# nicooff/omp_amg

Hardware: AMD Instinct MI355X
Metric: AMG setup rows/sec + RAP SpGEMM nnz/sec at 1/2/4/8 MI355X (higher is better)
Workload: dtype f64

## Files before the change

omp_amg_amd/__init__.py:

```python
from __future__ import annotations

import ctypes as C
import os
import subprocess

import numpy as np

from . import abi

HERE = os.path.dirname(os.path.abspath(__file__))
LIB_PATH = os.path.join(HERE, "libomp_amg_amd.so")
_lib = None


class AmgdStats(C.Structure):
    _fields_ = [("t_total_ms", C.c_double), ("t_build_ms", C.c_double),
                ("t_coarsen_ms", C.c_double), ("t_smoother_ms", C.c_double),
                ("t_interp_ms", C.c_double), ("t_rap_ms", C.c_double),
                ("t_copy_ms", C.c_double), ("rap_kernel_ms", C.c_double),
                ("rap_out_nnz", C.c_uint64), ("rap_bytes", C.c_uint64),
                ("rows0", C.c_uint64), ("nnz0", C.c_uint64),
                ("nlevels", C.c_uint32), ("ub_events", C.c_uint32),
                ("peak_bytes", C.c_size_t), ("spmv_kernel_ms", C.c_double),
                ("spmv_bytes", C.c_uint64), ("spmv_bytes_strict", C.c_uint64),
# ... 64 lines not shown
        L.amgd_test_kry_mdot_n.argtypes = [C.c_void_p, C.c_void_p, C.c_uint64, C.c_uint64, C.c_int, C.c_void_p,
                                           C.c_void_p]
        L.amgd_test_kry_update_n.argtypes = [C.c_void_p, C.c_void_p, C.c_void_p, C.c_uint64, C.c_uint64, C.c_int,
                                             C.c_void_p, C.c_void_p]
        L.amgd_test_kry_mdot.argtypes = [C.c_void_p, C.c_void_p, C.c_uint64, C.c_uint64, C.c_int, C.c_void_p]
        L.amgd_test_kry_update.argtypes = [C.c_void_p, C.c_void_p, C.c_void_p, C.c_uint64, C.c_uint64, C.c_int,
                                           C.c_void_p]
        L.amgd_test_vc_level_n.argtypes = [C.POINTER(HCsr), C.POINTER(HCsr), C.POINTER(HCsr), C.c_void_p,
                                           C.c_uint32, C.c_double, C.c_void_p, C.c_void_p, C.c_void_p,
                                           C.c_int, C.c_int]
        L.amgd_test_vc_restrict_n.argtypes = [C.POINTER(HCsr), C.c_void_p, C.c_void_p, C.c_int, C.c_int]
        L.amgd_test_vc_mrhs_k.argtypes = [C.c_int]
        L.amgd_test_vc_mrhs_family.argtypes = [C.c_int]
        L.amgd_test_vc_row_max.argtypes = [C.c_uint32]
        L.amgd_test_vc_level.argtypes = [C.POINTER(HCsr), C.POINTER(HCsr), C.POINTER(HCsr), C.c_void_p,
                                         C.c_uint32, C.c_double, C.c_void_p, C.c_void_p, C.c_int,
                                         C.c_void_p, C.c_void_p, C.c_void_p]
        L.amgd_test_vc_restrict.argtypes = [C.POINTER(HCsr), C.c_void_p, C.c_void_p, C.c_int]
        L.amgd_hier_rows.argtypes = [C.c_void_p, C.POINTER(C.c_uint32), C.POINTER(C.c_uint32)]
        L.amgd_hier_rows.restype = C.c_int
        L.amgd_solve_comm_stats.argtypes = [C.POINTER(C.c_uint64), C.POINTER(C.c_uint64)]
        L.amgd_test_vc_halo.argtypes = [C.c_int]
        L.amgd_test_vc_repl.argtypes = [C.c_int64]
        L.amgd_test_vc_restrict_map.argtypes = [C.POINTER(HCsr), C.c_void_p, C.c_void_p, C.c_uint32,
                                                C.c_void_p, C.c_int]
        L.amgd_test_vc_halo_xch.argtypes = [C.POINTER(HCsr), C.c_void_p, C.c_void_p, C.c_void_p]
        L.amgd_test_vc_fused.argtypes = [C.c_int]
        L.amgd_test_vc_tail.argtypes = [C.c_int]
        L.amgd_test_vc_coop.argtypes = [C.c_int]
        L.amgd_dev_alloc.argtypes = [C.c_size_t]
        L.amgd_dev_alloc.restype = C.c_void_p
        L.amgd_dev_free.argtypes = [C.c_void_p]
        L.amgd_dev_upload.argtypes = [C.c_void_p, C.c_void_p, C.c_size_t]
        L.amgd_dev_download.argtypes = [C.c_void_p, C.c_void_p, C.c_size_t]
        L.amgd_test_csr.argtypes = [C.c_int, C.POINTER(HCsr), C.POINTER(HCsr), C.c_double,
                                    C.c_double, C.POINTER(HCsr)]
        L.amgd_test_spmv.argtypes = [C.POINTER(HCsr), C.c_void_p, C.c_double, C.c_void_p,
                                     C.c_double, C.c_void_p]
        L.amgd_test_spmv_f.argtypes = [C.POINTER(HCsr), C.c_void_p, C.c_double, C.c_void_p,
                                       C.c_double, C.c_void_p, C.c_void_p]
        L.amgd_test_spmv_rows.argtypes = [C.POINTER(HCsr), C.c_void_p, C.c_uint32, C.c_void_p,
                                          C.c_void_p]
        L.amgd_test_spmv_sl_min.argtypes = [C.c_int64]
        L.amgd_test_build.argtypes = [C.c_uint64, C.c_void_p, C.c_void_p, C.c_void_p,
                                      C.POINTER(HCsr)]
        L.amgd_test_math.argtypes = [C.c_int, C.c_uint64, C.c_void_p, C.c_void_p, C.c_void_p]
        L.amgd_test_free.argtypes = [C.POINTER(HCsr)]
        L.amgd_test_dot.argtypes = [C.c_int, C.c_uint64, C.c_void_p, C.c_void_p, C.c_int, C.c_int]
        L.amgd_test_dot.restype = C.c_double
        L.amgd_test_lmop_mode.argtypes = [C.c_int]
        L.amgd_test_spgemm_flat.argtypes = [C.c_int]
        L.amgd_test_spgemm_win.argtypes = [C.c_int]
        L.amgd_test_qf_reuse.argtypes = [C.c_int]
        L.amgd_test_sg_pattern.argtypes = [C.c_int]
        L.amgd_test_lmop_wave.argtypes = [C.c_int]
        L.amgd_test_lmop_small.argtypes = [C.c_int]
        L.amgd_test_lmop_stats.argtypes = [C.POINTER(C.c_uint64), C.c_int]
        L.amgd_test_lmop_prune.argtypes = [C.c_int]
        L.amgd_test_qf_sparse.argtypes = [C.c_int]
        L.amgd_test_qf_stats.argtypes = [C.POINTER(C.c_uint64)]
        L.amgd_test_qf_coop_lds.argtypes = [C.c_int]
        L.amgd_test_qf_split.argtypes = [C.c_int]
        L.amgd_test_mv_long.argtypes = [C.c_int64]
        L.amgd_test_fs_long.argtypes = [C.c_int64]
        L.amgd_test_spmv_rw.argtypes = [C.c_int]
        L.amgd_test_spmv_pair.argtypes = [C.c_int]
        L.amgd_test_spmv_rw_bounds.argtypes = [C.c_int, C.c_int]
        L.amgd_test_d2h_poll.argtypes = [C.c_int]
        L.amgd_test_fs_amx.argtypes = [C.c_int]
        L.amgd_test_qa_tile.argtypes = [C.c_int]
        L.amgd_test_qa_huge.argtypes = [C.c_int]
        L.amgd_test_qa_small.argtypes = [C.c_int]
        L.amgd_test_spmv_shard_calls.restype = C.c_uint64
        L.amgd_test_route_stats.argtypes = [C.POINTER(C.c_uint64), C.c_int]
        L.amgd_comm_rccl_uid.argtypes = [C.c_char_p]
        L.amgd_comm_rccl_uid.restype = C.c_int
        L.amgd_comm_init_rccl.argtypes = [C.c_int, C.c_int, C.c_char_p]
        L.amgd_comm_init_rccl.restype = C.c_int
        L.amgd_comm_init_host.argtypes = [C.c_int, C.c_int, C.c_void_p, C.c_void_p]
        L.amgd_comm_init_host.restype = C.c_int
        L.amgd_comm_init_sim.argtypes = [C.c_int]
        L.amgd_comm_init_sim.restype = C.c_int
        L.amgd_comm_set_min_work.argtypes = [C.c_double]
        L.amgd_comm_stats.argtypes = [C.POINTER(C.c_uint64), C.POINTER(C.c_uint64),
                                      C.POINTER(C.c_double)]
        _lib = L
    return _lib


def init(device: int = 0) -> None:
    L = lib()
    if L.amgd_init(device) != 0:
        raise RuntimeError("omp_amg_amd: no usable HIP device: " + L.amgd_error().decode())


def amg_setup(Ai, Aj, Av, *, seed: int = 1) -> abi.Hierarchy:
    init()
    return abi.run_setup(lib(), Ai, Aj, Av, seed=seed, quiet=False)


def stats() -> dict:
    st = AmgdStats()
    lib().amgd_get_stats(C.byref(st))
    out = {}
    for f, _ in AmgdStats._fields_:
        v = getattr(st, f)
# ... 446 lines not shown

def lmop_stats(reset: bool = True) -> dict:
    out = (C.c_uint64 * 5)()
    lib().amgd_test_lmop_stats(out, int(reset))
    return {"fast": out[0], "general": out[1], "dirty_prefix": out[2], "misses": out[3],
            "pruned": out[4]}


def lmop_prune(n: int) -> None:
    lib().amgd_test_lmop_prune(int(n))


def spgemm_dr_sort(on: int) -> None:
    lib().amgd_test_spgemm_dr_sort(int(on))


def spat_inc(on: int) -> None:
    lib().amgd_test_spat_inc(int(on))


def skel_tr(on: int) -> None:
    lib().amgd_test_skel_tr(int(on))


def fuse_arr(on: int) -> None:
    lib().amgd_test_fuse_arr(int(on))


def spat_stats() -> dict:
    out = (C.c_uint64 * 3)()
    lib().amgd_test_spat_stats(out)
    return {"incremental": out[0], "whole": out[1], "same": out[2]}


def spgemm_sym(mode: int) -> None:
    lib().amgd_test_spgemm_sym(int(mode))


def spgemm_sym_stats() -> dict:
    L = lib()
    k, r = C.c_uint64(), C.c_uint64()
    L.amgd_test_spgemm_sym_stats(C.byref(k), C.byref(r))
    return {"kept": k.value, "reused": r.value}


def spgemm_win(w: int) -> None:
    lib().amgd_test_spgemm_win(int(w))


def qf_reuse(on: int) -> None:
    lib().amgd_test_qf_reuse(int(on))


def lmop_wave(n: int) -> None:
    lib().amgd_test_lmop_wave(int(n))


def sg_pattern(on: int) -> None:
    lib().amgd_test_sg_pattern(int(on))


def qa_small(on: int) -> None:
    lib().amgd_test_qa_small(int(on))


def lmop_qq_budget(nbytes: int) -> None:
    L = lib()
    L.amgd_test_lmop_qq_budget.argtypes = [C.c_int64]
    L.amgd_test_lmop_qq_budget(int(nbytes))


def _hcsr_any(M):
    h = _to_hcsr(M.row_off, M.col if len(M.col) else np.zeros(1), M.a if len(M.a) else np.zeros(1),
                 M.rn, M.cn)
    h.nnz = int(M.row_off[-1])
    return h


def test_qapply(Wt: abi.Csr, A: abi.Csr, Bt: abi.Csr, u, lam):
    init()
    L = lib()
    L.amgd_test_qapply.argtypes = [C.POINTER(HCsr), C.POINTER(HCsr), C.POINTER(HCsr), C.c_void_p,
                                   C.c_void_p, C.c_void_p]
    hs = [_hcsr_any(M) for M in (Wt, A, Bt)]
    u = np.ascontiguousarray(u, dtype=np.float64)
    lam = np.ascontiguousarray(lam, dtype=np.float64)
    assert len(u) == Wt.rn and len(lam) == Wt.cn
    out = np.zeros(int(Wt.row_off[-1]) + 1)
    rc = L.amgd_test_qapply(C.byref(hs[0]), C.byref(hs[1]), C.byref(hs[2]), u.ctypes.data,
                            lam.ctypes.data, out.ctypes.data)
    if rc != 0:
        raise RuntimeError(f"amgd_test_qapply failed rc={rc}")
    return out[:-1]


def test_lmop(S: abi.Csr, Wskel: abi.Csr, A: abi.Csr, u):
    init()
    L = lib()
    L.amgd_test_lmop.argtypes = [C.POINTER(HCsr), C.POINTER(HCsr), C.POINTER(HCsr), C.c_void_p,
                                 C.c_void_p]
    hs = [_hcsr_any(M) for M in (S, Wskel, A)]
    u = np.ascontiguousarray(u, dtype=np.float64)
    assert len(u) == Wskel.cn
    out = np.zeros(int(S.row_off[-1]) + 1)
    rc = L.amgd_test_lmop(C.byref(hs[0]), C.byref(hs[1]), C.byref(hs[2]), u.ctypes.data, out.ctypes.data)
    if rc != 0:
# ... 580 lines not shown
```

omp_amg_amd/csrc/amgd_interp.hip:

```cpp
#include <hip/hip_runtime.h>
#include <cstring>
#include <rocprim/device/device_radix_sort.hpp>

#include <cfloat>
#include <cstdio>
#include <cstdlib>
#include <algorithm>
#include <vector>

#include "amgd.h"
#include "amgd_dev.h"

__device__ __forceinline__ uint64_t tri(uint64_t i) { return i * (i + 1) / 2; }

__device__ __forceinline__ double row_lookup(const uint32_t *col, const double *a, uint64_t a0,
                                             uint64_t a1, uint32_t j) {
  uint64_t lo = a0, hi = a1;
  while (lo < hi) {
    uint64_t mid = (lo + hi) >> 1;
    if (col[mid] < j) lo = mid + 1;
    else hi = mid;
  }
  return (lo < a1 && col[lo] == j) ? a[lo] : 0.0;
}
// ... 161 lines not shown
#pragma unroll
    for (int q = 0; q < QB; q++) {
      uint32_t j = j0 + q;
      if (j < k && j >= i) y += r[q] * s2[j];
    }
  }
  return y;
}

__global__ __launch_bounds__(256) void k_qfactor_mid(const uint32_t *rows, uint32_t nrows,
                                                     const uint64_t *wro, const uint32_t *wcol,
                                                     const uint64_t *aro, const uint32_t *acol,
                                                     const double *aa, const uint64_t *qoff,
                                                     double *Q) {
  __shared__ double s1[1024], s2[1024], qk[1024];
  __shared__ uint32_t Qs[1024];
  __shared__ double sh_al;
  const int t = threadIdx.x, lane = t & 63;
  for (uint32_t r = blockIdx.x; r < nrows; r += gridDim.x) {
    const uint32_t c = rows[r];
    const uint64_t w0 = wro[c];
    const uint32_t nz = (uint32_t)(wro[c + 1] - w0);
    for (uint32_t m = t; m < nz; m += 256) Qs[m] = wcol[w0 + m];
    double *U = Q + qoff[c];
    __syncthreads();
    for (uint32_t k = 0; k < nz; k++) {
      const uint32_t sk = Qs[k];
      gather_s1<256>(s1, Qs, k, acol, aa, aro[sk], aro[sk + 1]);
      __syncthreads();
      for (uint32_t i = t; i < k; i += 256) s2[i] = seq_dot_batched(U + tri(i), s1, i + 1);
      __syncthreads();
      for (uint32_t ib = t - lane; ib < k; ib += 256) {
        const uint32_t i = ib + lane;
        double y = mv_ut_lane(U, s2, ib, i, k);
        if (i < k) qk[i] = y;
      }
      __syncthreads();
      if (t == 0) {
        double al = s1[k];
        for (uint32_t m = 0; m < k; m++) al -= s1[m] * qk[m];
        sh_al = -1.0 / sqrt(al);
      }
      __syncthreads();
      const double al = sh_al;
      double *out = U + tri(k);
      for (uint32_t i = t; i < k; i += 256) out[i] = qk[i] * al;
      if (t == 0) out[k] = -al;
      __syncthreads();
    }
  }
}

#define QB2 16
template <int NZMAX, int B, int NTT = 256>
__global__ __launch_bounds__(NTT) void k_qfactor_blk(const uint32_t *rows, uint32_t nrows,
                                                     const uint64_t *wro, const uint32_t *wcol,
                                                     const uint64_t *aro, const uint32_t *acol,
                                                     const double *aa, const uint64_t *qoff,
                                                     double *Q) {
  constexpr uint32_t NT = NTT, RPT = (NZMAX + NT - 1) / NT, PAD = NZMAX + 16;
  __shared__ uint32_t Qs[NZMAX];
  __shared__ double S1[B * PAD], S2[B * PAD], qk[PAD];
  __shared__ double sh_al;
  const uint32_t t = threadIdx.x, lane = t & 63;
  for (uint32_t r = blockIdx.x; r < nrows; r += gridDim.x) {
    const uint32_t c = rows[r];
    const uint64_t w0 = wro[c];
    const uint32_t nz = (uint32_t)(wro[c + 1] - w0);
    for (uint32_t m = t; m < nz; m += NT) Qs[m] = wcol[w0 + m];
    double *U = Q + qoff[c];
    __syncthreads();
    for (uint32_t k0 = 0; k0 < nz; k0 += B) {
      const uint32_t bn = min((uint32_t)B, nz - k0);
      for (uint32_t b = 0; b < bn; b++)
        for (uint32_t m = t; m <= k0 + b; m += NT) S1[b * PAD + m] = 0.0;
      uint64_t ra0[B];
      uint32_t rlen[B], spre[B + 1], lpre[B + 1];
      uint32_t look_cost = 0, scan_cost = 0;
      spre[0] = lpre[0] = 0;
#pragma unroll
      for (int b = 0; b < B; b++) {
        ra0[b] = 0;
        rlen[b] = 0;
        if ((uint32_t)b < bn) {
          const uint32_t k = k0 + b, sk = Qs[k];
          ra0[b] = aro[sk];
          rlen[b] = (uint32_t)(aro[sk + 1] - ra0[b]);
          const uint32_t lg_len = 32 - __clz(rlen[b] | 1), lg_k = 32 - __clz(k + 1);
          look_cost += (k + 1) * lg_len * 4;
          scan_cost += rlen[b] * (4 + lg_k);
        }
        spre[b + 1] = spre[b] + rlen[b];
        lpre[b + 1] = lpre[b] + ((uint32_t)b < bn ? k0 + b + 1 : 0u);
      }
      __syncthreads();
      if (look_cost < scan_cost) {
        for (uint32_t fl = t; fl < lpre[B]; fl += NT) {
          uint32_t b = 0;
#pragma unroll
          for (int q = 1; q < B; q++) b += fl >= lpre[q] ? 1u : 0u;
          const uint32_t m = fl - lpre[b];
          S1[b * PAD + m] = row_lookup(acol, aa, ra0[b], ra0[b] + rlen[b], Qs[m]);
        }
      } else {
        for (uint32_t fl = t; fl < spre[B]; fl += NT) {
          uint32_t b = 0;
#pragma unroll
          for (int q = 1; q < B; q++) b += fl >= spre[q] ? 1u : 0u;
          const uint64_t a0 = ra0[b], e = a0 + (fl - spre[b]);
          const uint32_t k = k0 + b;
          const uint32_t j = acol[e];
          if (e > a0 && acol[e - 1] == j) continue;
          uint32_t lo = 0, hi = k + 1;
          while (lo < hi) {
            const uint32_t mid = (lo + hi) >> 1;
            if (Qs[mid] < j) lo = mid + 1;
            else hi = mid;
          }
          if (lo <= k && Qs[lo] == j) S1[b * PAD + lo] = aa[e];
        }
      }
      __syncthreads();
      for (uint32_t i = t; i < k0; i += NT) {
        double acc[B];
#pragma unroll
        for (int b = 0; b < B; b++) acc[b] = 0.0;
        const double *Ui = U + tri(i);
        for (uint32_t j0 = 0; j0 <= i; j0 += QB2) {
          double u[QB2];
#pragma unroll
          for (int q = 0; q < QB2; q++) u[q] = (j0 + q <= i) ? Ui[j0 + q] : 0.0;
#pragma unroll
          for (int q = 0; q < QB2; q++)
            if (j0 + q <= i) {
#pragma unroll
              for (int b = 0; b < B; b++) acc[b] += u[q] * S1[b * PAD + j0 + q];
            }
        }
#pragma unroll
        for (int b = 0; b < B; b++)
          if ((uint32_t)b < bn) S2[b * PAD + i] = acc[b];
      }
      __syncthreads();
      double part[RPT][B];
#pragma unroll
      for (uint32_t rr = 0; rr < RPT; rr++) {
        const uint32_t ib = (t - lane) + rr * NT, i = ib + lane;
#pragma unroll
        for (int b = 0; b < B; b++) part[rr][b] = 0.0;
        for (uint32_t j0 = ib; j0 < k0; j0 += QB2) {
          double u[QB2];
#pragma unroll
          for (int q = 0; q < QB2; q++) {
            const uint32_t j = j0 + q;
            u[q] = (j < k0 && j >= i) ? U[tri(j) + i] : 0.0;
          }
#pragma unroll
          for (int q = 0; q < QB2; q++) {
            const uint32_t j = j0 + q;
            if (j < k0 && j >= i) {
#pragma unroll
              for (int b = 0; b < B; b++) part[rr][b] += u[q] * S2[b * PAD + j];
            }
          }
        }
      }
#pragma unroll
      for (int b = 0; b < B; b++) {
        if ((uint32_t)b < bn) {
          const uint32_t k = k0 + b;
#pragma unroll
          for (uint32_t rr = 0; rr < RPT; rr++) {
            const uint32_t i = t + rr * NT;
            if (i < k) {
              double y = i < k0 ? part[rr][b] : 0.0;
              for (uint32_t j = max(i, k0); j < k; j++) y += U[tri(j) + i] * S2[b * PAD + j];
              qk[i] = y;
            }
          }
          __syncthreads();
          if (t == 0) {
            const double *s1 = S1 + b * PAD;
            double al = s1[k];
            for (uint32_t m0 = 0; m0 < k; m0 += LB) {
              double x[LB], y[LB];
#pragma unroll
              for (int q = 0; q < LB; q++) { x[q] = s1[m0 + q]; y[q] = qk[m0 + q]; }
#pragma unroll
              for (int q = 0; q < LB; q++)
                if (m0 + q < k) al -= x[q] * y[q];
            }
            sh_al = -1.0 / sqrt(al);
          }
          __syncthreads();
          const double al = sh_al;
          double *out = U + tri(k);
          for (uint32_t i = t; i < k; i += NT) out[i] = qk[i] * al;
          if (t == 0) out[k] = -al;
          if (t < bn - 1 - b) {
            const double *s1 = S1 + (b + 1 + t) * PAD;
            double v = 0;
            for (uint32_t j0 = 0; j0 < k; j0 += LB) {
              double x[LB], y[LB];
#pragma unroll
              for (int q = 0; q < LB; q++) { x[q] = qk[j0 + q]; y[q] = s1[j0 + q]; }
#pragma unroll
              for (int q = 0; q < LB; q++)
                if (j0 + q < k) v += (x[q] * al) * y[q];
            }
            v += (-al) * s1[k];
            S2[(b + 1 + t) * PAD + k] = v;
          }
          __syncthreads();
        }
      }
    }
  }
}

__device__ __forceinline__ void grid_sync(unsigned *bar, unsigned nblocks, unsigned &gen) {
  __threadfence();
  __syncthreads();
  if (threadIdx.x == 0) {
    unsigned a = atomicAdd(&bar[0], 1u);
    if (a == nblocks - 1) {
      atomicExch(&bar[0], 0u);
      __threadfence();
      atomicAdd(&bar[1], 1u);
    } else {
      while (__hip_atomic_load(&bar[1], __ATOMIC_ACQUIRE, __HIP_MEMORY_SCOPE_AGENT) == gen)
        __builtin_amdgcn_s_sleep(1);
    }
  }
  __syncthreads();
  __threadfence();
  gen++;
}

#define QF_COOP_MAX 8192
template <bool LDS>
__global__ __launch_bounds__(64) void k_qfactor_coop(uint32_t c, const uint64_t *wro,
                                                     const uint32_t *wcol, const uint64_t *aro,
                                                     const uint32_t *acol, const double *aa,
                                                     const uint64_t *qoff, double *Q,
                                                     double *s1b, double *s2, double *qk,
                                                     unsigned *bar) {
  extern __shared__ double xs[];
  __shared__ double sh_al;
  const uint32_t lane = threadIdx.x, G = gridDim.x;
  const uint32_t gt = blockIdx.x * 64 + lane, GT = G * 64;
  const uint64_t w0 = wro[c];
  const uint32_t nz = (uint32_t)(wro[c + 1] - w0);
  const uint32_t *Qj = wcol + w0;
  double *U = Q + qoff[c];
  double *xa = xs, *xb = xs + nz;
  unsigned gen = 0;
  for (uint32_t k = 0; k <= nz; k++) {
    if (k > 0) {
      const uint32_t kp = k - 1;
      const double *s1p = s1b + (uint64_t)(kp & 1) * nz;
      if (LDS) {
// ... 233 lines not shown
}
__global__ void k_max_nz(const uint64_t *wro, uint32_t rn, unsigned long long *mx) {
  unsigned long long m = 0;
  GRID_STRIDE(c, rn) m = max(m, (unsigned long long)(wro[c + 1] - wro[c]));
  atomicMax(mx, m);
}

struct RowSplit {
  uint32_t *sl, *bl;
  unsigned ns, nb;
  uint64_t maxnz;
};
static RowSplit split_rows(const dcsr *Wt, uint32_t cap, uint32_t cb, uint32_t ce) {
  RowSplit rs;
  const uint64_t L = (uint64_t)Wt->rn + 1;
  rs.sl = (uint32_t *)amgd_alloc(2 * L * 4);
  rs.bl = rs.sl + L;
  unsigned *cnt = (unsigned *)amgd_alloc(32);
  amgd_memset(cnt, 0, 32);
  if (ce > cb) {
    k_bin_nz<<<grid_for(ce - cb), 256, 0, amgd_s()>>>(Wt->ro, cb, ce, BinLim{{cap}}, 2, rs.sl, cnt, L);
    k_max_nz<<<grid_for(Wt->rn), 256, 0, amgd_s()>>>(Wt->ro, Wt->rn, (unsigned long long *)(cnt + 4));
  }
  unsigned h[8];
  amgd_d2h(h, cnt, 32);
  amgd_free(cnt);
  rs.ns = h[0];
  rs.nb = h[1];
  uint64_t mx;
  memcpy(&mx, &h[4], 8);
  rs.maxnz = mx;
  return rs;
}
static void free_split(RowSplit &rs) { amgd_free(rs.sl); }

static int g_qf_sparse = -1;
static bool g_qf_sparse_forced = false;
static int qf_sparse_mode() {
  if (g_qf_sparse < 0) {
    const char *e = getenv("AMGD_QF_SPARSE");
    g_qf_sparse = e ? atoi(e) : 1;
    g_qf_sparse_forced = e != nullptr;
  }
  return g_qf_sparse;
}
static int qf_blocked() {
  static int b = -1;
  if (b < 0) {
    const char *e = getenv("AMGD_QF_BLOCKED");
    b = e ? atoi(e) : 1;
  }
  return b;
}
static uint32_t g_coop_lds_max = QF_COOP_MAX;
extern "C" void amgd_qfactor_set_coop_lds(int m) { g_coop_lds_max = m < 0 ? QF_COOP_MAX : (uint32_t)m; }
static unsigned long g_qf_stats[3];
extern "C" void amgd_qfactor_set_sparse(int m) {
  g_qf_sparse = m;
  g_qf_sparse_forced = m >= 0 && m != 1;
}
extern "C" void amgd_qfactor_stats(unsigned long *st) {
  st[0] = g_qf_stats[0];
  st[1] = g_qf_stats[1];
  st[2] = g_qf_stats[2];
  g_qf_stats[0] = g_qf_stats[1] = g_qf_stats[2] = 0;
}
#define QF_T0 32
#define QF_T1 64
#define QF_T2 128
#define QF_T3 1024
__global__ void k_cc_init(const uint32_t *Qj, uint32_t nz, uint32_t *pos, uint32_t *lab) {
  GRID_STRIDE(k, nz) {
    pos[Qj[k]] = (uint32_t)k;
    lab[k] = (uint32_t)k;
  }
}
__global__ void k_cc_reset(const uint32_t *Qj, uint32_t nz, uint32_t *pos) {
  GRID_STRIDE(k, nz) pos[Qj[k]] = 0xffffffffu;
}
__global__ void k_cc_hook(const uint32_t *Qj, uint32_t nz, const uint64_t *aro,
                          const uint32_t *acol, const uint32_t *pos, uint32_t *lab,
                          unsigned *changed) {
  GRID_STRIDE(k, nz) {
    const uint32_t r = Qj[k];
    uint32_t m = lab[k];
    for (uint64_t e = aro[r]; e < aro[r + 1]; e++) {
      const uint32_t p = pos[acol[e]];
      if (p != 0xffffffffu) m = min(m, lab[p]);
    }
    bool ch = false;
    for (uint64_t e = aro[r]; e < aro[r + 1]; e++) {
      const uint32_t p = pos[acol[e]];
      if (p == 0xffffffffu) continue;
      const uint32_t lp = lab[p];
      if (m < lp) { atomicMin(&lab[lp], m); atomicMin(&lab[p], m); ch = true; }
    }
    const uint32_t lk = lab[k];
    if (m < lk) { atomicMin(&lab[lk], m); atomicMin(&lab[k], m); ch = true; }
    if (ch) *changed = 1u;
  }
}
__global__ void k_cc_init_iota(uint32_t nz, uint32_t *lab) { GRID_STRIDE(k, nz) lab[k] = (uint32_t)k; }
__global__ void k_cc_jump(uint32_t nz, uint32_t *lab) {
  GRID_STRIDE(k, nz) {
    uint32_t l = lab[k];
    while (lab[l] != l) l = lab[l];
// ... 248 lines not shown
      return g_qf_split_depth > 0 && nz <= 8192 && !g_qf_sparse_forced ? 0 : sp0;
    };
    std::vector<uint32_t> bigs;
    for (uint32_t c : big) {
      const uint32_t nz = (uint32_t)(ro[c + 1] - ro[c]);
      if (!qfactor_split(c, Wt, A, ro[c], nz, Q + qo[c])) bigs.push_back(c);
    }
    big.swap(bigs);
    if (!big.empty()) amgd_sync();
    for (uint32_t c : big) {
      uint32_t nz = (uint32_t)(ro[c + 1] - ro[c]);
      bignz.push_back(nz);
      const int sp = sp_of(nz);
      if (!sp) {
        bigstat.push_back(nullptr);
        launch_coop(c, nz);
        continue;
      }
      const uint64_t tn = (uint64_t)nz * (nz + 1) / 2;
      const uint32_t cap = sp == 2 ? nz + 8 : (uint32_t)std::min<uint64_t>(tn, 1u << 24);
      const size_t nd = (size_t)nz * 3 + cap, nu = (size_t)nz * 6 + (size_t)cap * 3 + 2;
      char *mem = (char *)amgd_alloc(nd * 8 + nu * 4 + 64);
      coop_bufs.push_back(mem);
      QsBuf qb;
      qb.s1 = (double *)mem;
      qb.s2 = qb.s1 + nz;
      qb.qk = qb.s2 + nz;
      qb.uval = qb.qk + nz;
      uint32_t *u = (uint32_t *)(qb.uval + cap);
      qb.m2 = u;
      qb.m3 = u + nz;
      qb.L2 = u + 2 * (size_t)nz;
      qb.chead = u + 3 * (size_t)nz;
      qb.ctail = u + 4 * (size_t)nz;
      qb.rowptr = u + 5 * (size_t)nz;
      qb.ucol = u + 6 * (size_t)nz + 1;
      qb.urow = qb.ucol + cap;
      qb.nxt = qb.urow + cap;
      qb.status = qb.nxt + cap;
      qb.cap = cap;
      HIPCK(hipMemsetAsync(mem, 0, (size_t)nz * 3 * 8, s2));
      HIPCK(hipMemsetAsync(qb.m2, 0, (size_t)nz * 3 * 4, s2));
      HIPCK(hipMemsetAsync(qb.chead, 0xff, (size_t)nz * 2 * 4, s2));
      k_fill_negzero<<<grid_for(tn), 256, 0, s2>>>(Q + qo[c], tn);
      k_qfactor_sparse<256><<<1, 256, 0, s2>>>(c, Wt->ro, Wt->col, A->ro, A->col, A->a, qoff, Q, qb);
      KCHECK();
      bigstat.push_back(qb.status);
    }
    HIPCK(hipEventRecord(ev2, s2));
  }
  if (hn[0])
    k_qfactor_lds<QF_T0, 64><<<(int)std::min<unsigned>(hn[0], 65536u), 64, 0, s>>>(
        lists, hn[0], Wt->ro, Wt->col, A->ro, A->col, A->a, qoff, Q);
  if (hn[1])
    k_qfactor_blk<QF_T1, 4, 64><<<(int)std::min<unsigned>(hn[1], 65536u), 64, 0, s>>>(
        lists + L, hn[1], Wt->ro, Wt->col, A->ro, A->col, A->a, qoff, Q);
  if (hn[2])
    k_qfactor_blk<QF_T2, 4, 128><<<(int)std::min<unsigned>(hn[2], 65536u), 128, 0, s>>>(
        lists + 2 * L, hn[2], Wt->ro, Wt->col, A->ro, A->col, A->a, qoff, Q);
  if (qf_blocked()) {
    if (hn[3])
      k_qfactor_blk<256, 4><<<(int)std::min<unsigned>(hn[3], 8192u), 256, 0, s>>>(
          lists + 3 * L, hn[3], Wt->ro, Wt->col, A->ro, A->col, A->a, qoff, Q);
    if (hn[4]) amgd_route_hit(AMGD_R_QF_T512);
    if (hn[5]) amgd_route_hit(AMGD_R_QF_T1024);
    if (hn[4])
      k_qfactor_blk<512, 4><<<(int)std::min<unsigned>(hn[4], 8192u), 256, 0, s>>>(
          lists + 4 * L, hn[4], Wt->ro, Wt->col, A->ro, A->col, A->a, qoff, Q);
    if (hn[5])
      k_qfactor_blk<QF_T3, 4><<<(int)std::min<unsigned>(hn[5], 8192u), 256, 0, s>>>(
          lists + 5 * L, hn[5], Wt->ro, Wt->col, A->ro, A->col, A->a, qoff, Q);
  } else {
    for (int q = 3; q < 6; q++)
      if (hn[q])
        k_qfactor_mid<<<(int)std::min<unsigned>(hn[q], 8192u), 256, 0, s>>>(
            lists + q * L, hn[q], Wt->ro, Wt->col, A->ro, A->col, A->a, qoff, Q);
  }
  KCHECK();
  if (hn[HUGE]) {
    bool redo = false;
    for (size_t q = 0; q < big.size(); q++) {
      if (!bigstat[q]) continue;
      unsigned st = 0;
      HIPCK(hipMemcpyAsync(&st, bigstat[q], 4, hipMemcpyDeviceToHost, s2));
      HIPCK(hipStreamSynchronize(s2));
      if (st) {
        amgd_sync();
        launch_coop(big[q], bignz[q]);
        redo = true;
      }
      g_qf_stats[st ? 1 : 0]++;
    }
    if (redo) HIPCK(hipEventRecord(ev2, s2));
    HIPCK(hipStreamWaitEvent(s, ev2, 0));
    for (void *p : coop_bufs) amgd_free(p);
  }
  if (sglog) {
    amgd_sync();
    fprintf(stderr, "qfactor cols %u nnz %lu tiers %u/%u/%u/%u/%u/%u/%u (huge nz %u) Q %lu  %.2f ms\n",
            rn, (unsigned long)Wt->nnz, hn[0], hn[1], hn[2], hn[3], hn[4], hn[5], hn[6],
            bignz.empty() ? 0u : bignz[0], (unsigned long)tot, (amgd_wtime() - t_start) * 1e3);
  }
  amgd_free(lists); amgd_free(cnt);
}

__global__ void k_qcost(const uint64_t *wro, uint32_t rn, uint64_t *cost, const uint8_t *skip) {
  GRID_STRIDE(c, rn) {
    uint64_t nz = wro[c + 1] - wro[c];
    cost[c] = (skip && skip[c] ? nz * nz / 8 : nz <= 1024 ? nz * nz * nz : nz * nz * 1024) + 1;
  }
}
#define QF_SHARD_MIN (1ull << 30)
static int g_qf_reuse = -1;
static int qf_reuse_on() {
  if (g_qf_reuse < 0) { const char *e = getenv("AMGD_QF_REUSE"); g_qf_reuse = e && *e ? atoi(e) : 1; }
  return g_qf_reuse;
}
extern "C" void amgd_qfactor_set_reuse(int on) { g_qf_reuse = on < 0 ? -1 : on; }
extern "C" void amgd_qfactor_reuse_stats(uint64_t *reused, uint64_t *factored) {
  *reused = g_qf_reused; *factored = g_qf_factored;
}
extern "C" double *amgd_qfactor(const dcsr *Wt, const dcsr *A, uint64_t **qoff_out,
                                uint64_t *qtotal) {
  return amgd_qfactor_reuse(Wt, A, qoff_out, qtotal, nullptr, nullptr, nullptr);
}
extern "C" double *amgd_qfactor_reuse(const dcsr *Wt, const dcsr *A, uint64_t **qoff_out,
                                      uint64_t *qtotal, const dcsr *Wp, const double *Qp,
                                      const uint64_t *qpoff) {
  hipStream_t s = amgd_s();
  const uint32_t rn = Wt->rn;
// ... 1575 lines not shown
```

omp_amg_amd/csrc/amgd_testapi.c:

```c
#include <stdlib.h>
#include <string.h>

#include "amgd.h"

#define API __attribute__((visibility("default")))

typedef struct { uint32_t rn, cn; uint64_t nnz; uint64_t *ro; uint32_t *col; double *a; } hcsr;

static dcsr *up(const hcsr *H) {
  dcsr *A = dcsr_new(H->rn, H->cn, H->nnz);
  amgd_h2d(A->ro, H->ro, ((size_t)H->rn + 1) * 8);
  amgd_h2d(A->col, H->col, H->nnz * 4);
  amgd_h2d(A->a, H->a, H->nnz * 8);
  return A;
}
static void down(const dcsr *A, hcsr *H) {
  H->rn = A->rn; H->cn = A->cn; H->nnz = A->nnz;
  H->ro = (uint64_t *)malloc(((size_t)A->rn + 1) * 8);
  H->col = (uint32_t *)malloc(A->nnz * 4 + 4);
  H->a = (double *)malloc(A->nnz * 8 + 8);
  amgd_d2h(H->ro, A->ro, ((size_t)A->rn + 1) * 8);
  amgd_d2h(H->col, A->col, A->nnz * 4);
  amgd_d2h(H->a, A->a, A->nnz * 8);
}
// ... 152 lines not shown

extern void amgd_set_seq_plain(int on);
API double amgd_test_dot(int mode, uint64_t n, const double *a, const double *b, int plain, int exact) {
  if (amgd_rt_init(0) != 0) return 0.0 / 0.0;
  double *da = (double *)amgd_alloc(n * 8 + 8), *db = (double *)amgd_alloc(n * 8 + 8);
  amgd_h2d(da, a, n * 8);
  amgd_h2d(db, b, n * 8);
  int old = amgd_get_exact();
  amgd_set_exact(exact);
  amgd_set_seq_plain(plain);
  double r = mode == 0 ? amgd_dot(da, db, n) : mode == 1 ? amgd_dot(da, NULL, n) : amgd_dot3(da, db, n);
  amgd_set_seq_plain(0);
  amgd_set_exact(old);
  amgd_free(da); amgd_free(db);
  return r;
}

API void amgd_test_free(hcsr *H) {
  free(H->ro); free(H->col); free(H->a);
  H->ro = NULL; H->col = NULL; H->a = NULL;
}

API void amgd_test_lmop_mode(int m) { amgd_lmop_set_mode(m); }
extern void amgd_lmop_set_prune(int n);
API void amgd_test_lmop_prune(int n) { amgd_lmop_set_prune(n); }
API void amgd_test_lmop_stats(uint64_t *out, int reset) {
  amgd_lmop_stats(out);
  if (reset) amgd_lmop_stats_reset();
}

API void amgd_test_qf_sparse(int m) { amgd_qfactor_set_sparse(m); }
API void amgd_test_qf_stats(uint64_t *out) {
  unsigned long st[3];
  amgd_qfactor_stats(st);
  out[0] = st[0];
  out[1] = st[1];
  out[2] = st[2];
}

extern uint64_t amgd_spmv_shard_calls(void);
API int amgd_test_cols_masked(const hcsr *HA, const uint8_t *hmask, hcsr *HX) {
  if (amgd_rt_init(0) != 0) return -1;
  dcsr *A = up(HA);
  uint8_t *m = (uint8_t *)amgd_alloc((size_t)A->cn + 1);
  amgd_h2d(m, hmask, A->cn);
  dcsr *X = amgd_cols_masked(A, m);
  down(X, HX);
  dcsr_free(&X); dcsr_free(&A);
  amgd_free(m);
  return 0;
}
void amgd_qfactor_set_reuse(int on);
API void amgd_test_qf_reuse(int on) { amgd_qfactor_set_reuse(on); }
void amgd_lmop_set_small(int n);
API void amgd_test_lmop_small(int n) { amgd_lmop_set_small(n); }
void amgd_lmop_set_wave(int n);
API void amgd_test_lmop_wave(int n) { amgd_lmop_set_wave(n); }
void amgd_spgemm_set_pattern(int on);
API void amgd_test_sg_pattern(int on) { amgd_spgemm_set_pattern(on); }
API void amgd_test_qf_reuse_stats(uint64_t *out) {
  static uint64_t r0 = 0, f0 = 0;
  uint64_t r, f;
  amgd_qfactor_reuse_stats(&r, &f);
  out[0] = r - r0; out[1] = f - f0;
  r0 = r; f0 = f;
}
API void amgd_test_hbm_cap(uint64_t bytes) { amgd_set_hbm_cap((size_t)bytes); }
API uint64_t amgd_test_pool_inuse(void) { return amgd_pool_bytes_in_use(); }

API int amgd_test_comm(int kind, uint64_t bytes, uint64_t expect) {
  const int N = amgd_pcomm_size(), me = amgd_pcomm_rank();
  uint64_t *so = (uint64_t *)malloc(8 * ((size_t)N + 1)), *ro = (uint64_t *)malloc(8 * ((size_t)N + 1));
  for (int p = 0; p <= N; p++) { so[p] = bytes * p; ro[p] = (kind ? expect : bytes) * p; }
  char *sb = (char *)amgd_alloc(bytes * N + 16), *rb = (char *)amgd_alloc(ro[N] + 16);
  amgd_memset(sb, me + 1, bytes * N);
  if (kind == 0) {
    void *b = sb;
    amgd_allgatherv(1, &b, so);
  } else {
    amgd_pcomm_alltoallv(sb, so, rb, ro);
  }
  amgd_sync();
  amgd_free(sb); amgd_free(rb);
  free(so); free(ro);
  return 0;
}
API void amgd_test_route_stats(uint64_t *out, int reset) {
  for (int r = 0; r < AMGD_R_N; r++) out[r] = amgd_route_ctr[r];
  if (reset) memset(amgd_route_ctr, 0, sizeof amgd_route_ctr);
}
API uint64_t amgd_test_spmv_shard_calls(void) { return amgd_spmv_shard_calls(); }

extern void amgd_qapply_set_huge(int n);
API void amgd_test_qa_huge(int n) { amgd_qapply_set_huge(n); }
extern void amgd_spmv_set_rw(int rw);
API void amgd_test_spmv_rw(int rw) { amgd_spmv_set_rw(rw); }
extern void amgd_spmv_set_pair(int on);
extern void amgd_spmv_set_rw_bounds(int lo, int hi);
extern void amgd_set_d2h_poll(int on);
extern void amgd_fs_set_amx(int on);
API void amgd_test_fs_amx(int on) { amgd_fs_set_amx(on); }
extern void amgd_qa_set_tile(int t);
API void amgd_test_qa_tile(int t) { amgd_qa_set_tile(t); }
API void amgd_test_d2h_poll(int on) { amgd_set_d2h_poll(on); }
API void amgd_test_part_stats(uint64_t *out) {
  amgd_part_stats(out);
// ... 834 lines not shown
```

Measured before the change: 713,000.

## Pipeline LDS dot chains and keep own Q columns in registers in qfactor

The blocked Q-factor kernel gets a software-pipelined LDS dot-product helper that loads the next batch while it accumulates the current one. It keeps each thread's newly computed U entries in registers, so the intra-block updates stop re-reading U from global memory. For the 512 and 1024 buckets it adds a pass_terms helper that handles full 16-wide panels without predicates, using wave-uniform bounds from readfirstlane, with optional lookahead loads. Both paths are on by default behind env and test switches, and a grid-size override is added. The cost is more registers and template instantiations, plus reads past k that rely on the padding.

Result: faster. 726,600, median of 6 (+1.9%).

```diff
diff --git a/omp_amg_amd/__init__.py b/omp_amg_amd/__init__.py
--- a/omp_amg_amd/__init__.py
+++ b/omp_amg_amd/__init__.py
@@ -140,6 +140,9 @@
         L.amgd_test_spgemm_flat.argtypes = [C.c_int]
         L.amgd_test_spgemm_win.argtypes = [C.c_int]
         L.amgd_test_qf_reuse.argtypes = [C.c_int]
+        L.amgd_test_qf_chain.argtypes = [C.c_int]
+        L.amgd_test_qf_pass.argtypes = [C.c_int]
+        L.amgd_test_qf_grid.argtypes = [C.c_int]
         L.amgd_test_sg_pattern.argtypes = [C.c_int]
         L.amgd_test_lmop_wave.argtypes = [C.c_int]
         L.amgd_test_lmop_small.argtypes = [C.c_int]
@@ -692,6 +695,18 @@
     lib().amgd_test_qf_reuse(int(on))
 
 
+def qf_chain(on: int) -> None:
+    lib().amgd_test_qf_chain(int(on))
+
+
+def qf_pass(on: int) -> None:
+    lib().amgd_test_qf_pass(int(on))
+
+
+def qf_grid(n: int) -> None:
+    lib().amgd_test_qf_grid(int(n))
+
+
 def lmop_wave(n: int) -> None:
     lib().amgd_test_lmop_wave(int(n))
 
diff --git a/omp_amg_amd/csrc/amgd_interp.hip b/omp_amg_amd/csrc/amgd_interp.hip
--- a/omp_amg_amd/csrc/amgd_interp.hip
+++ b/omp_amg_amd/csrc/amgd_interp.hip
@@ -237,13 +237,74 @@
 }
 
 #define QB2 16
-template <int NZMAX, int B, int NTT = 256>
+template <int L, bool SUB>
+__device__ __forceinline__ double lds_chain_ahead(const double *x, const double *y, uint32_t n,
+                                                  double acc, double al) {
+  static_assert(L <= 9 || L == 16, "reads stay inside the 16-element padding");
+  double p[L];
+#pragma unroll
+  for (int q = 0; q < L; q++) p[q] = SUB ? x[q] * y[q] : (x[q] * al) * y[q];
+  for (uint32_t m0 = 0; m0 < n; m0 += L) {
+    double nx[L], ny[L];
+#pragma unroll
+    for (int q = 0; q < L; q++) { nx[q] = x[m0 + L + q]; ny[q] = y[m0 + L + q]; }
+#pragma unroll
+    for (int q = 0; q < L; q++)
+      if (m0 + q < n) {
+        if (SUB) acc -= p[q];
+        else acc += p[q];
+      }
+#pragma unroll
+    for (int q = 0; q < L; q++) p[q] = SUB ? nx[q] * ny[q] : (nx[q] * al) * ny[q];
+  }
+  return acc;
+}
+template <int N, int G, bool AHEAD, int B, uint32_t PAD, bool PRED>
+__device__ __forceinline__ void pass_terms(double (&acc)[B], const double (&u)[N], const double *X,
+                                           int lo, int hi) {
+  static_assert(N % G == 0, "whole groups");
+  double x[G][B];
+#pragma unroll
+  for (int g = 0; g < G; g++)
+#pragma unroll
+    for (int b = 0; b < B; b++) x[g][b] = X[b * PAD + g];
+#pragma unroll
+  for (int q0 = 0; q0 < N; q0 += G) {
+    double nx[G][B];
+    if (AHEAD && q0 + G < N) {
+#pragma unroll
+      for (int g = 0; g < G; g++)
+#pragma unroll
+        for (int b = 0; b < B; b++) nx[g][b] = X[b * PAD + q0 + G + g];
+    }
+#pragma unroll
+    for (int g = 0; g < G; g++) {
+      const int q = q0 + g;
+      if (!PRED || (q >= lo && q < hi)) {
+#pragma unroll
+        for (int b = 0; b < B; b++) acc[b] += u[q] * x[g][b];
+      }
+    }
+    __builtin_amdgcn_sched_barrier(0);
+    if (q0 + G < N) {
+#pragma unroll
+      for (int g = 0; g < G; g++)
+#pragma unroll
+        for (int b = 0; b < B; b++) x[g][b] = AHEAD ? nx[g][b] : X[b * PAD + q0 + G + g];
+    }
+  }
+}
+template <int NZMAX, int B, int NTT = 256, bool CH = true, bool PS = true>
 __global__ __launch_bounds__(NTT) void k_qfactor_blk(const uint32_t *rows, uint32_t nrows,
                                                      const uint64_t *wro, const uint32_t *wcol,
                                                      const uint64_t *aro, const uint32_t *acol,
                                                      const double *aa, const uint64_t *qoff,
                                                      double *Q) {
   constexpr uint32_t NT = NTT, RPT = (NZMAX + NT - 1) / NT, PAD = NZMAX + 16;
+  constexpr int LC = NZMAX >= 1024 ? 16 : NZMAX >= 512 ? 8 : 6;
+  static_assert(LC <= 9 || NZMAX % 16 == 0, "chain reads one batch past k stay inside PAD");
+  constexpr int PG = 4;
+  constexpr bool PA = NZMAX >= 1024;
   __shared__ uint32_t Qs[NZMAX];
   __shared__ double S1[B * PAD], S2[B * PAD], qk[PAD];
   __shared__ double sh_al;
@@ -311,16 +372,32 @@
 #pragma unroll
         for (int b = 0; b < B; b++) acc[b] = 0.0;
         const double *Ui = U + tri(i);
-        for (uint32_t j0 = 0; j0 <= i; j0 += QB2) {
-          double u[QB2];
-#pragma unroll
-          for (int q = 0; q < QB2; q++) u[q] = (j0 + q <= i) ? Ui[j0 + q] : 0.0;
-#pragma unroll
-          for (int q = 0; q < QB2; q++)
-            if (j0 + q <= i) {
-#pragma unroll
-              for (int b = 0; b < B; b++) acc[b] += u[q] * S1[b * PAD + j0 + q];
+        if (PS) {
+          const uint32_t ib = __builtin_amdgcn_readfirstlane(i - lane);
+          for (uint32_t j0 = 0; j0 <= i; j0 += QB2) {
+            double u[QB2];
+            if (j0 + QB2 - 1 <= ib) {
+#pragma unroll
+              for (int q = 0; q < QB2; q++) u[q] = Ui[j0 + q];
+              pass_terms<QB2, PG, PA, B, PAD, false>(acc, u, S1 + j0, 0, 0);
+            } else {
+#pragma unroll
+              for (int q = 0; q < QB2; q++) u[q] = (j0 + q <= i) ? Ui[j0 + q] : 0.0;
+              pass_terms<QB2, PG, PA, B, PAD, true>(acc, u, S1 + j0, 0, (int)(i - j0) + 1);
             }
+          }
+        } else {
+          for (uint32_t j0 = 0; j0 <= i; j0 += QB2) {
+            double u[QB2];
+#pragma unroll
+            for (int q = 0; q < QB2; q++) u[q] = (j0 + q <= i) ? Ui[j0 + q] : 0.0;
+#pragma unroll
+            for (int q = 0; q < QB2; q++)
+              if (j0 + q <= i) {
+#pragma unroll
+                for (int b = 0; b < B; b++) acc[b] += u[q] * S1[b * PAD + j0 + q];
+              }
+          }
         }
 #pragma unroll
         for (int b = 0; b < B; b++)
@@ -330,68 +407,118 @@
       double part[RPT][B];
 #pragma unroll
       for (uint32_t rr = 0; rr < RPT; rr++) {
-        const uint32_t ib = (t - lane) + rr * NT, i = ib + lane;
+        const uint32_t ib = __builtin_amdgcn_readfirstlane((t - lane) + rr * NT), i = ib + lane;
 #pragma unroll
         for (int b = 0; b < B; b++) part[rr][b] = 0.0;
         for (uint32_t j0 = ib; j0 < k0; j0 += QB2) {
           double u[QB2];
-#pragma unroll
-          for (int q = 0; q < QB2; q++) {
-            const uint32_t j = j0 + q;
-            u[q] = (j < k0 && j >= i) ? U[tri(j) + i] : 0.0;
-          }
-#pragma unroll
-          for (int q = 0; q < QB2; q++) {
-            const uint32_t j = j0 + q;
-            if (j < k0 && j >= i) {
-#pragma unroll
-              for (int b = 0; b < B; b++) part[rr][b] += u[q] * S2[b * PAD + j];
+          if (PS && j0 >= ib + 64 && j0 + QB2 <= k0) {
+#pragma unroll
+            for (int q = 0; q < QB2; q++) u[q] = U[tri(j0 + q) + i];
+            pass_terms<QB2, PG, PA, B, PAD, false>(part[rr], u, S2 + j0, 0, 0);
+          } else if (PS) {
+#pragma unroll
+            for (int q = 0; q < QB2; q++) {
+              const uint32_t j = j0 + q;
+              u[q] = (j < k0 && j >= i) ? U[tri(j) + i] : 0.0;
+            }
+            pass_terms<QB2, PG, PA, B, PAD, true>(part[rr], u, S2 + j0, (int)i - (int)j0, (int)(k0 - j0));
+          } else {
+#pragma unroll
+            for (int q = 0; q < QB2; q++) {
+              const uint32_t j = j0 + q;
+              u[q] = (j < k0 && j >= i) ? U[tri(j) + i] : 0.0;
+            }
+#pragma unroll
+            for (int q = 0; q < QB2; q++) {
+              const uint32_t j = j0 + q;
+              if (j < k0 && j >= i) {
+#pragma unroll
+                for (int b = 0; b < B; b++) part[rr][b] += u[q] * S2[b * PAD + j];
+              }
             }
           }
         }
       }
+      double own[RPT][B];
+#pragma unroll
+      for (uint32_t rr = 0; rr < RPT; rr++)
+#pragma unroll
+        for (int b = 0; b < B; b++) own[rr][b] = 0.0;
 #pragma unroll
       for (int b = 0; b < B; b++) {
         if ((uint32_t)b < bn) {
           const uint32_t k = k0 + b;
+          double yk[RPT];
 #pragma unroll
           for (uint32_t rr = 0; rr < RPT; rr++) {
             const uint32_t i = t + rr * NT;
+            yk[rr] = 0.0;
             if (i < k) {
               double y = i < k0 ? part[rr][b] : 0.0;
-              for (uint32_t j = max(i, k0); j < k; j++) y += U[tri(j) + i] * S2[b * PAD + j];
+              if (CH) {
+#pragma unroll
+                for (int bp = 0; bp < b; bp++)
+                  if (k0 + bp >= i) y += own[rr][bp] * S2[b * PAD + k0 + bp];
+              } else {
+                for (uint32_t j = max(i, k0); j < k; j++) y += U[tri(j) + i] * S2[b * PAD + j];
+              }
               qk[i] = y;
+              yk[rr] = y;
             }
           }
           __syncthreads();
           if (t == 0) {
             const double *s1 = S1 + b * PAD;
             double al = s1[k];
-            for (uint32_t m0 = 0; m0 < k; m0 += LB) {
-              double x[LB], y[LB];
-#pragma unroll
-              for (int q = 0; q < LB; q++) { x[q] = s1[m0 + q]; y[q] = qk[m0 + q]; }
-#pragma unroll
-              for (int q = 0; q < LB; q++)
-                if (m0 + q < k) al -= x[q] * y[q];
+            if (CH) {
+              al = lds_chain_ahead<LC, true>(s1, qk, k, al, 0.0);
+            } else {
+              for (uint32_t m0 = 0; m0 < k; m0 += LB) {
+                double x[LB], y[LB];
+#pragma unroll
+                for (int q = 0; q < LB; q++) { x[q] = s1[m0 + q]; y[q] = qk[m0 + q]; }
+#pragma unroll
+                for (int q = 0; q < LB; q++)
+                  if (m0 + q < k) al -= x[q] * y[q];
+              }
             }
             sh_al = -1.0 / sqrt(al);
           }
           __syncthreads();
           const double al = sh_al;
           double *out = U + tri(k);
-          for (uint32_t i = t; i < k; i += NT) out[i] = qk[i] * al;
-          if (t == 0) out[k] = -al;
+          if (CH) {
+#pragma unroll
+            for (uint32_t rr = 0; rr < RPT; rr++) {
+              const uint32_t i = t + rr * NT;
+              if (i < k) {
+                const double u = yk[rr] * al;
+                out[i] = u;
+                own[rr][b] = u;
+              } else if (i == k) {
+                out[k] = -al;
+                own[rr][b] = -al;
+              }
+            }
+          } else {
+            for (uint32_t i = t; i < k; i += NT) out[i] = qk[i] * al;
+            if (t == 0) out[k] = -al;
+          }
           if (t < bn - 1 - b) {
             const double *s1 = S1 + (b + 1 + t) * PAD;
             double v = 0;
-            for (uint32_t j0 = 0; j0 < k; j0 += LB) {
-              double x[LB], y[LB];
-#pragma unroll
-              for (int q = 0; q < LB; q++) { x[q] = qk[j0 + q]; y[q] = s1[j0 + q]; }
-#pragma unroll
-              for (int q = 0; q < LB; q++)
-                if (j0 + q < k) v += (x[q] * al) * y[q];
+            if (CH) {
+              v = lds_chain_ahead<LC, false>(qk, s1, k, v, al);
+            } else {
+              for (uint32_t j0 = 0; j0 < k; j0 += LB) {
+                double x[LB], y[LB];
+#pragma unroll
+                for (int q = 0; q < LB; q++) { x[q] = qk[j0 + q]; y[q] = s1[j0 + q]; }
+#pragma unroll
+                for (int q = 0; q < LB; q++)
+                  if (j0 + q < k) v += (x[q] * al) * y[q];
+              }
             }
             v += (-al) * s1[k];
             S2[(b + 1 + t) * PAD + k] = v;
@@ -731,6 +858,20 @@
   }
   return b;
 }
+static int g_qf_chain = -1;
+static int qf_chain() {
+  if (g_qf_chain < 0) { const char *e = getenv("AMGD_QF_CHAIN"); g_qf_chain = e && *e ? atoi(e) : 1; }
+  return g_qf_chain;
+}
+extern "C" void amgd_qfactor_set_chain(int on) { g_qf_chain = on; }
+static int g_qf_pass = -1;
+static int qf_pass() {
+  if (g_qf_pass < 0) { const char *e = getenv("AMGD_QF_PASS"); g_qf_pass = e && *e ? atoi(e) : 1; }
+  return g_qf_pass;
+}
+extern "C" void amgd_qfactor_set_pass(int on) { g_qf_pass = on; }
+static int g_qf_grid = 0;
+extern "C" void amgd_qfactor_set_grid(int n) { g_qf_grid = n > 0 ? n : 0; }
 static uint32_t g_coop_lds_max = QF_COOP_MAX;
 extern "C" void amgd_qfactor_set_coop_lds(int m) { g_coop_lds_max = m < 0 ? QF_COOP_MAX : (uint32_t)m; }
 static unsigned long g_qf_stats[3];
@@ -1085,30 +1226,42 @@
   if (hn[0])
     k_qfactor_lds<QF_T0, 64><<<(int)std::min<unsigned>(hn[0], 65536u), 64, 0, s>>>(
         lists, hn[0], Wt->ro, Wt->col, A->ro, A->col, A->a, qoff, Q);
-  if (hn[1])
-    k_qfactor_blk<QF_T1, 4, 64><<<(int)std::min<unsigned>(hn[1], 65536u), 64, 0, s>>>(
-        lists + L, hn[1], Wt->ro, Wt->col, A->ro, A->col, A->a, qoff, Q);
-  if (hn[2])
-    k_qfactor_blk<QF_T2, 4, 128><<<(int)std::min<unsigned>(hn[2], 65536u), 128, 0, s>>>(
-        lists + 2 * L, hn[2], Wt->ro, Wt->col, A->ro, A->col, A->a, qoff, Q);
+  const bool ch = qf_chain() != 0, ps = qf_pass() != 0;
+  auto blk_grid = [&](unsigned n, unsigned cap) {
+    return (int)std::min<unsigned>(n, g_qf_grid > 0 ? (unsigned)g_qf_grid : cap);
+  };
+#define QF_BLK1(NZ, NTH, q, cap, CHV, PSV)                                                   \
+  k_qfactor_blk<NZ, 4, NTH, CHV, PSV><<<blk_grid(hn[q], cap), NTH, 0, s>>>(                  \
+      lists + (q) * L, hn[q], Wt->ro, Wt->col, A->ro, A->col, A->a, qoff, Q)
+#define QF_BLK(NZ, NTH, q, cap)                                                              \
+  do {                                                                                       \
+    if (ch && ps) QF_BLK1(NZ, NTH, q, cap, true, true);                                      \
+    else if (ch) QF_BLK1(NZ, NTH, q, cap, true, false);                                      \
+    else if (ps) QF_BLK1(NZ, NTH, q, cap, false, true);                                      \
+    else QF_BLK1(NZ, NTH, q, cap, false, false);                                             \
+  } while (0)
+#define QF_BLK_S(NZ, NTH, q, cap)                \
+  do {                                                                                       \
+    if (ch) QF_BLK1(NZ, NTH, q, cap, true, false);                                           \
+    else QF_BLK1(NZ, NTH, q, cap, false, false);                                             \
+  } while (0)
+  if (hn[1]) QF_BLK_S(QF_T1, 64, 1, 65536u);
+  if (hn[2]) QF_BLK_S(QF_T2, 128, 2, 65536u);
   if (qf_blocked()) {
-    if (hn[3])
-      k_qfactor_blk<256, 4><<<(int)std::min<unsigned>(hn[3], 8192u), 256, 0, s>>>(
-          lists + 3 * L, hn[3], Wt->ro, Wt->col, A->ro, A->col, A->a, qoff, Q);
+    if (hn[3]) QF_BLK_S(256, 256, 3, 8192u);
     if (hn[4]) amgd_route_hit(AMGD_R_QF_T512);
     if (hn[5]) amgd_route_hit(AMGD_R_QF_T1024);
-    if (hn[4])
-      k_qfactor_blk<512, 4><<<(int)std::min<unsigned>(hn[4], 8192u), 256, 0, s>>>(
-          lists + 4 * L, hn[4], Wt->ro, Wt->col, A->ro, A->col, A->a, qoff, Q);
-    if (hn[5])
-      k_qfactor_blk<QF_T3, 4><<<(int)std::min<unsigned>(hn[5], 8192u), 256, 0, s>>>(
-          lists + 5 * L, hn[5], Wt->ro, Wt->col, A->ro, A->col, A->a, qoff, Q);
+    if (hn[4]) QF_BLK(512, 256, 4, 8192u);
+    if (hn[5]) QF_BLK(QF_T3, 256, 5, 8192u);
   } else {
     for (int q = 3; q < 6; q++)
       if (hn[q])
         k_qfactor_mid<<<(int)std::min<unsigned>(hn[q], 8192u), 256, 0, s>>>(
             lists + q * L, hn[q], Wt->ro, Wt->col, A->ro, A->col, A->a, qoff, Q);
   }
+#undef QF_BLK
+#undef QF_BLK_S
+#undef QF_BLK1
   KCHECK();
   if (hn[HUGE]) {
     bool redo = false;
diff --git a/omp_amg_amd/csrc/amgd_testapi.c b/omp_amg_amd/csrc/amgd_testapi.c
--- a/omp_amg_amd/csrc/amgd_testapi.c
+++ b/omp_amg_amd/csrc/amgd_testapi.c
@@ -228,6 +228,12 @@
 }
 void amgd_qfactor_set_reuse(int on);
 API void amgd_test_qf_reuse(int on) { amgd_qfactor_set_reuse(on); }
+void amgd_qfactor_set_chain(int on);
+API void amgd_test_qf_chain(int on) { amgd_qfactor_set_chain(on); }
+void amgd_qfactor_set_pass(int on);
+API void amgd_test_qf_pass(int on) { amgd_qfactor_set_pass(on); }
+void amgd_qfactor_set_grid(int n);
+API void amgd_test_qf_grid(int n) { amgd_qfactor_set_grid(n); }
 void amgd_lmop_set_small(int n);
 API void amgd_test_lmop_small(int n) { amgd_lmop_set_small(n); }
 void amgd_lmop_set_wave(int n);
```
